# ukeSJTU/tiaozhanbei-unet

Measured on AMD Instinct MI355X. Metric: training images/sec, AnomalyUNet 256x256 bs=32 per GPU, higher is better.
Workload: dtype bf16; 1 GPU; AnomalyUNet 3x256x256, bs=32/GPU, MSE+focal loss, Adam (BASELINE.json configs[2], synthetic randn images, bernoulli masks); global_batch=32, parallelism=dp1, accumulate=fp32, master_params=fp32, dist_world=1, reserved_cus=0, cu_budget=256

## Files before the change

### tiaozhanbei_unet_amd/csrc/igemm.hip

```cpp
#include <stdlib.h>

#include <type_traits>

#include "common.h"

namespace {

struct DView { const char* p; int C, H, W, oy, ox; };
struct DViewW { char* p; int C, H, W, oy, ox; };

struct IgemmParams {
  DView src[2];
  DViewW dst[2];
  int N, H, W;
  int Ctot;
  int Cout;
  int wK;
  const char* w;
  const float* bias;
  int dst_split;
  int accumulate;
  int relu;
  int imul, gtaps;
  int omul, nZ;
  int zdiv;
  float* stats;
  int tilesX, tilesY, nCo;
  const char* bn_y;
  const float* bn_scale;
  const float* bn_shift;
  const float* bn_mean;
  int co_il;
  int pdma_stagger;
  int pdma_dense;
  int pdma_dense_src;
};

constexpr int TH = 8, TW = 16, NPIX = TH * TW;

template <typename T, int TAPS, int BN, int KG>
struct Cfg {
  static constexpr int R = (TAPS == 9) ? 3 : 1;
  static constexpr int HH = TH + R - 1, HW = TW + R - 1;
  static constexpr int CHB = KG * 32;
  static constexpr int PSTR = CHB + 16;
  static constexpr int PPP = CHB / 16;
  static constexpr int A_BUFS = (TAPS == 1) ? 2 : 1;
  static constexpr int A_BYTES = HH * HW * PSTR;
  static constexpr int B_BYTES = BN * PSTR;
  static constexpr int LDS = A_BUFS * A_BYTES + 2 * B_BYTES;
  static constexpr int CK = KG * ET<T>::KGC;
  static constexpr int WCO = BN / 64, WPX = 4 / WCO, PXT = NPIX / (32 * WPX);
  static constexpr int NAP = (HH * HW * PPP + 255) / 256;
  static constexpr int NBP = (BN * PPP + 255) / 256;
  static constexpr bool BN_PIECES_EXACT = (BN * PPP) % 256 == 0;
};

template <typename T, int TAPS, int BN, int KG>
__global__ __launch_bounds__(256, 2) void igemm_kernel(const IgemmParams P) {
  using C = Cfg<T, TAPS, BN, KG>;
  using E = ET<T>;
  extern __shared__ __attribute__((aligned(16))) char smem[];
  char* const sA = smem;
  char* const sB = smem + C::A_BUFS * C::A_BYTES;

  const int tid = threadIdx.x, lane = tid & 63, wave = tid >> 6;
  const int wco = wave % C::WCO, wpx = wave / C::WCO;
  const int l31 = lane & 31, hh = lane >> 5;

  int logical;
  {
    const int total = gridDim.x, b = blockIdx.x;
    const int xcd = b & 7, slot = b >> 3, q = total >> 3, r = total & 7;
    logical = (xcd < r ? xcd * (q + 1) : r * (q + 1) + (xcd - r) * q) + slot;
  }
  const int cot = logical % P.nCo;
  int t = logical / P.nCo;
  const int z = t % P.nZ;  t /= P.nZ;
  const int txi = t % P.tilesX;  t /= P.tilesX;
  const int tyi = t % P.tilesY;
  const int n = t / P.tilesY;
  const int ty0 = tyi * TH, tx0 = txi * TW;
  const int co0 = cot * BN;

  f32x16 acc[2][C::PXT];
#pragma unroll
  for (int a = 0; a < 2; ++a)
#pragma unroll
    for (int b = 0; b < C::PXT; ++b)
#pragma unroll
      for (int r = 0; r < 16; ++r) acc[a][b][r] = 0.f;

  int aoff[2];
#pragma unroll
  for (int ct = 0; ct < 2; ++ct) aoff[ct] = (wco * 64 + ct * 32 + l31) * C::PSTR + hh * 16;
  int boff[C::PXT];
#pragma unroll
  for (int pt = 0; pt < C::PXT; ++pt) {
    const int m = wpx * (32 * C::PXT) + pt * 32 + l31;
    boff[pt] = ((m >> 4) * C::HW + (m & 15)) * C::PSTR + hh * 16;
  }

  const int cpt = P.Ctot / C::CK;
  const int nchunks = P.gtaps * cpt;

  u32x4 breg[C::NBP];
  auto load_b = [&](int tap, int chunk) {
#pragma unroll
    for (int i = 0; i < C::NBP; ++i) {
      const int id = tid + i * 256;
      if (C::BN_PIECES_EXACT || id < BN * C::PPP) {
        const int row = id / C::PPP, part = id % C::PPP;
        const size_t e = ((size_t)((z * TAPS + tap) * P.Cout + co0 + row)) * P.wK + (size_t)chunk * C::CK;
        breg[i] = *reinterpret_cast<const u32x4*>(P.w + e * E::ES + part * 16);
      }
    }
  };
  auto store_b = [&](int buf) {
// ... 642 lines not shown
#pragma unroll
        for (int j = 0; j < 4; ++j) {
          const int cl = wco * 64 + ct * 16 + kb * 4 + j;
          red[(wpx * 2 + 0) * BN + cl] = bs[ct][j];
          red[(wpx * 2 + 1) * BN + cl] = bq[ct][j];
        }
    }
    __syncthreads();
    const int part = (n * P.tilesY + tyi) * P.tilesX + txi;
    for (int i = tid; i < 2 * BN; i += 256) {
      const int q = i / BN, cl = i - q * BN;
      float t = 0.f;
#pragma unroll
      for (int wp = 0; wp < C::WPX; ++wp) t += red[(wp * 2 + q) * BN + cl];
      P.stats[((size_t)part * 2 + q) * P.Cout + co0 + cl] = t;
    }
  }
}

template <typename T, int BN, int KG>
int32_t launch3(const IgemmParams& Pin, int kclass, hipStream_t s, int* stat_parts) {
  using C = Cfg3<T, BN, KG>;
  IgemmParams P = Pin;
  const long long blocks = (long long)P.N * P.tilesY * P.tilesX * P.nCo;
  UNET_REQUIRE(blocks > 0 && blocks < (1LL << 31), UNET_ERR_UNSUPPORTED, "conv3: grid of %lld blocks", blocks);
  const double flops = 2.0 * P.N * P.H * P.W * (double)P.Cout * P.Ctot * 9;
  if constexpr (sizeof(T) == 2 && BN == 128 && KG == 4) {
    using CM = Cfg3M<T, BN, KG>;
    auto km = conv3m16_kernel<T, BN, KG>;
    unet_set_max_lds(reinterpret_cast<const void*>(km), CM::LDS);
    if (P.stats && stat_parts) *stat_parts = P.N * P.tilesY * P.tilesX;
    ProfScope prof(kclass, flops, s, "conv3m16_kernel");
    hipLaunchKernelGGL(km, dim3((unsigned)blocks), dim3(256), CM::LDS, s, P);
    return unet_check_launch("conv3m16_kernel");
  } else {
    auto kern = conv3_kernel<T, BN, KG>;
    unet_set_max_lds(reinterpret_cast<const void*>(kern), C::LDS);
    P.stats = nullptr;
    ProfScope prof(kclass, flops, s, "conv3_kernel");
    hipLaunchKernelGGL(kern, dim3((unsigned)blocks), dim3(256), C::LDS, s, P);
    return unet_check_launch("conv3_kernel");
  }
}

template <int N>
__device__ __forceinline__ void row16_sum_n(float (&v)[N]) {
  static_assert(N >= 3, "hazard distance");
  asm volatile("s_nop 1");
#pragma unroll
  for (int i = 0; i < N; ++i)
    asm volatile("v_add_f32_dpp %0, %1, %1 quad_perm:[1,0,3,2] row_mask:0xf bank_mask:0xf" : "=v"(v[i]) : "0"(v[i]));
#pragma unroll
  for (int i = 0; i < N; ++i)
    asm volatile("v_add_f32_dpp %0, %1, %1 quad_perm:[2,3,0,1] row_mask:0xf bank_mask:0xf" : "=v"(v[i]) : "0"(v[i]));
#pragma unroll
  for (int i = 0; i < N; ++i)
    asm volatile("v_add_f32_dpp %0, %1, %1 row_half_mirror row_mask:0xf bank_mask:0xf" : "=v"(v[i]) : "0"(v[i]));
#pragma unroll
  for (int i = 0; i < N; ++i)
    asm volatile("v_add_f32_dpp %0, %1, %1 row_mirror row_mask:0xf bank_mask:0xf" : "=v"(v[i]) : "0"(v[i]));
}

__device__ __forceinline__ void pdma_item(int wk, int n_tiles, int c, int& cot, int& tile) {
  const int span = c * n_tiles;
  const int sg = wk / span, rem = wk - sg * span;
  tile = rem / c;
  cot = sg * c + (rem - tile * c);
}

template <int BN, bool PAIR = false>
struct CfgP {
  static constexpr int TH = 16, TW = 16, HH = 18, HW = 18;
  static constexpr int PSTR = 160, PPP = 10, RS = HW * PSTR;
  static constexpr int A_INSTR = (HH * HW * PPP + 63) / 64;
  static constexpr int A_BYTES = A_INSTR * 1024;
  static constexpr int NDA = (A_INSTR + 7) / 8;
  static constexpr int W_BYTES = (PAIR ? 2 : 1) * BN * 128, NDW = W_BYTES / 1024 / 8;
  static constexpr int NSLOT = 3;
  static constexpr int W_BASE = 0;
  static constexpr int A_BASE = NSLOT * W_BYTES;
  static constexpr int RED_BASE = A_BASE + 2 * A_BYTES;
  static constexpr int RED_BYTES = 4 * 2 * BN * 4;
  static constexpr int DUMMY = RED_BASE + RED_BYTES;
  static constexpr int LDS = DUMMY + 1024;
  static constexpr int CT = BN / 32;
  static constexpr int NST = CT / 2 * 4;
};

#ifndef PDMA_DEFER128
#define PDMA_DEFER128 (!PP && !BNBWD)
#endif
template <int BN, bool BNBWD = false, bool PP = false, bool PAIR = false>
__device__ __forceinline__ void conv3_pdma_body(const IgemmParams& P) {
  static_assert(!PAIR || (BN == 64 && !PP), "pair steps: the lock-step 64-channel kernel");
  using C = CfgP<BN, PAIR>;
  extern __shared__ __attribute__((aligned(16))) char smem[];
  typedef __attribute__((address_space(3))) void lds_void;
  constexpr unsigned OOB = 0xFFFFFFF0u;

  const int tid = threadIdx.x, lane = tid & 63, wave = tid >> 6;
  const int grp = wave >> 2;
  const int wco = PP ? grp : (wave & 1), wpx = PP ? (wave & 3) : (wave >> 1);
  const int l15 = lane & 15, kb = lane >> 4;

  const int G = gridDim.x;
  const int tiles_img = P.tilesY * P.tilesX;
  const int n_tiles = P.N * tiles_img;
  const int total = n_tiles * P.nCo;
  const int logical = (blockIdx.x & 7) * (G >> 3) + (blockIdx.x >> 3);
  if (logical >= total) return;

  int aoff[C::CT][2], boff[4];
#pragma unroll
  for (int ct = 0; ct < C::CT; ++ct) {
    const int row = wco * (BN / 2) + ct * 16 + l15;
#pragma unroll
    for (int ks = 0; ks < 2; ++ks) aoff[ct][ks] = row * 128 + (((ks * 4 + kb) ^ ((row >> 1) & 7)) << 4);
  }
#pragma unroll
  for (int pt = 0; pt < 4; ++pt) boff[pt] = (wpx * 4 + pt) * C::RS + l15 * C::PSTR + kb * 16;

  int a_code[C::NDA];
#pragma unroll
  for (int j = 0; j < C::NDA; ++j) {
    const int q = (j * 8 + wave) * 64 + lane;
    const int pix = q / C::PPP, part = q - pix * C::PPP;
    const int hy = pix / C::HW, hx = pix - hy * C::HW;
    const int edge = (hy == 0) | ((hy == C::HH - 1) << 1) | ((hx == 0) << 2) | ((hx == C::HW - 1) << 3);
    a_code[j] = (pix < C::HH * C::HW && part < 8) ? (hy | (hx << 8) | (part << 16) | (edge << 24)) : -1;
  }
  unsigned w_g[C::NDW];
#pragma unroll
  for (int j = 0; j < C::NDW; ++j) {
    const int q = (j * 8 + wave) * 64 + lane;
    const int row = q >> 3, pos = q & 7;
    w_g[j] = (unsigned)((row * P.wK) * 2 + ((pos ^ ((row >> 1) & 7)) << 4));
  }

  const int nchunks = P.Ctot / 64;
  const unsigned w_tap_stride = (unsigned)P.Cout * P.wK * 2;
  const __amdgpu_buffer_rsrc_t w_rsrc =
      __builtin_amdgcn_make_buffer_rsrc((void*)P.w, (short)0, (int)(9u * w_tap_stride), 0x00020000);
  const unsigned img0 = (unsigned)P.src[0].H * P.src[0].W * P.src[0].C * 2;
  const unsigned img1 = (unsigned)P.src[1].H * P.src[1].W * P.src[1].C * 2;

  unsigned a_g[2][C::NDA];
  __amdgpu_buffer_rsrc_t a_rsrc[2];
  unsigned d_wbase = 0;
  bool d_live = true;
  const bool dsrc = P.pdma_dense_src != 0;
  if (dsrc) {
#pragma unroll
    for (int j = 0; j < C::NDA; ++j) {
      const int code = a_code[j];
      const int hy = code & 255, hx = (code >> 8) & 255, part = (code >> 16) & 255;
      a_g[1][j] = code >= 0 ? (unsigned)(((hy * P.src[0].W + hx) * P.src[0].C) * 2 + part * 16) : OOB;
    }
  }
  auto setup_dma = [&](int wk) {
    int cot, tile;
    pdma_item(wk, n_tiles, P.co_il, cot, tile);
    const int n = tile / tiles_img, r = tile - n * tiles_img;
    const int ty0 = (r / P.tilesX) * C::TH, tx0 = (r % P.tilesX) * C::TW;
    d_wbase = (unsigned)(cot * BN) * P.wK * 2;
    if (dsrc) {
      const unsigned E = (unsigned)((ty0 == 0) | ((ty0 + C::TH == P.H) << 1) | ((tx0 == 0) << 2) | ((tx0 + C::TW == P.W) << 3)) << 24;
      const long long tb = ((long long)(ty0 - 1) * P.src[0].W + (tx0 - 1)) * (P.src[0].C * 2);
      a_rsrc[0] = __builtin_amdgcn_make_buffer_rsrc((void*)(P.src[0].p + (long long)n * img0 + tb), (short)0, 0x7FFFFFF0, 0x00020000);
      a_rsrc[1] = __builtin_amdgcn_make_buffer_rsrc((void*)(P.src[1].p ? P.src[1].p + (long long)n * img1 + tb : P.src[0].p),
                                                    (short)0, P.src[1].p ? 0x7FFFFFF0 : 0, 0x00020000);
#pragma unroll
      for (int j = 0; j < C::NDA; ++j) a_g[0][j] = ((unsigned)a_code[j] & E) ? OOB : a_g[1][j];
      return;
// ... 114 lines not shown
#pragma unroll
    for (int pt = 0; pt < 4; ++pt) f0[pt] = rb(pbA, 0, pt);
    const bf16x8 a0 = ra(0, 0, 0), a1 = ra(0, 0, 1);
    __builtin_amdgcn_sched_barrier(0);
#pragma unroll
    for (int pt = 0; pt < 4; ++pt) f1[pt] = rb(pbA, 1, pt);
    const bf16x8 a2 = ra(0, 1, 0), a3 = ra(0, 1, 1);
    mm(0, a0, f0);
    mm(1, a1, f0);
    __builtin_amdgcn_sched_barrier(0);
#pragma unroll
    for (int pt = 0; pt < 4; ++pt) g0[pt] = rb(pbB, 0, pt);
    const bf16x8 c0 = ra(1, 0, 0), c1 = ra(1, 0, 1);
    mm(0, a2, f1);
    mm(1, a3, f1);
    __builtin_amdgcn_sched_barrier(0);
#pragma unroll
    for (int pt = 0; pt < 4; ++pt) g1[pt] = rb(pbB, 1, pt);
    const bf16x8 c2 = ra(1, 1, 0), c3 = ra(1, 1, 1);
    mm(0, c0, g0);
    mm(1, c1, g0);
    __builtin_amdgcn_sched_barrier(0);
    mm(0, c2, g1);
    mm(1, c3, g1);
  };

  bf16x8 fa[2][C::CT], fb[2][4];
  auto load_frags = [&](int pbuf, int toff, int slot) {
    const char* pa = smem + C::W_BASE + slot * C::W_BYTES;
    const char* pb = smem + pbuf + toff;
#pragma unroll
    for (int ks = 0; ks < 2; ++ks) {
#pragma unroll
      for (int pt = 0; pt < 4; ++pt) fb[ks][pt] = *reinterpret_cast<const bf16x8*>(pb + boff[pt] + ks * 64);
#pragma unroll
      for (int ct = 0; ct < C::CT; ++ct) fa[ks][ct] = *reinterpret_cast<const bf16x8*>(pa + aoff[ct][ks]);
    }
  };
  auto mma_frags = [&]() {
#pragma unroll
    for (int ks = 0; ks < 2; ++ks)
#pragma unroll
      for (int ct = 0; ct < C::CT; ++ct)
#pragma unroll
        for (int pt = 0; pt < 4; ++pt)
          acc[ct][pt] = __builtin_amdgcn_mfma_f32_16x16x32_bf16(fa[ks][ct], fb[ks][pt], acc[ct][pt], 0, 0, 0);
  };

  setup_dma(logical);
#pragma unroll
  for (int j = 0; j < C::NDA; ++j) dma_patch(0, j, 0, true);
  if constexpr (PAIR) {
    dma_w2(d_wbase, 0, 0, true);
    dma_w2(d_wbase, 2, 1, true);
  } else {
    dma_w(d_wbase, 0, 0, 0, true);
    dma_w(d_wbase, 0, 1, 1, true);
  }
  if constexpr (PP) {
    asm volatile("s_waitcnt vmcnt(%0)" ::"n"(C::NDW) : "memory");
    __builtin_amdgcn_s_barrier();
    if (grp) __builtin_amdgcn_s_barrier();
  }

#ifdef PDMA_STAMPS
  unsigned long long st_sum[4] = {0, 0, 0, 0}, st_prev = 0, st_taps = 0, st_epi = 0, st_b2 = 0, st_rd = 0;
  const unsigned long long st_t0 = __builtin_amdgcn_s_memtime(), st_r0 = __builtin_amdgcn_s_memrealtime();
#endif
  int pbuf_i = 0;
  bool after_epilogue = false;
  const bool late_dma = !PP && P.pdma_stagger && __builtin_amdgcn_readfirstlane(wave) < 4;
  constexpr bool DEFER = BN == 64 || PDMA_DEFER128;
  const bool dense = BNBWD || P.pdma_dense != 0;
  unsigned lp[2];
#pragma unroll
  for (int q = 0; q < 2; ++q)
    lp[q] = (unsigned)((((wpx * 4) * P.dst[q].W + l15) * P.dst[q].C + (kb & 1) * 16 + (kb >> 1) * 8) * 2);
  float stat_tot = 0.f;
  float bs[C::CT][4], bq[C::CT][4];
#pragma unroll
  for (int ct = 0; ct < C::CT; ++ct)
#pragma unroll
    for (int j = 0; j < 4; ++j) { bs[ct][j] = 0.f; bq[ct][j] = 0.f; }
  for (int wk = logical; wk < total; wk += G) {
    int cot, tile;
    pdma_item(wk, n_tiles, P.co_il, cot, tile);
    const int n = tile / tiles_img, r = tile - n * tiles_img;
    const int tyi = r / P.tilesX, txi = r - tyi * P.tilesX;
    const int ty0 = tyi * C::TH, tx0 = txi * C::TW;
    const int co0 = cot * BN;
    const unsigned c_wbase = d_wbase;
    const bool has_next = wk + G < total;
#pragma unroll
    for (int a = 0; a < C::CT; ++a)
#pragma unroll
      for (int b = 0; b < 4; ++b)
#pragma unroll
        for (int q = 0; q < 4; ++q) acc[a][b][q] = 0.f;

    if constexpr (PAIR) {
#pragma unroll
      for (int d = 0; d < 9; ++d) {
        constexpr int NPIECE[9] = {2, 2, 2, 1, 0, 2, 2, 2, 1};
        if (d == 5) {
          d_live = has_next;
          if (has_next) setup_dma(wk + G);
        }
        if (d == 0) {
          if (after_epilogue) {
            if (P.stats) asm volatile("s_waitcnt vmcnt(%0)" ::"n"(C::NDW + C::NST + 1) : "memory");
            else asm volatile("s_waitcnt vmcnt(%0)" ::"n"(C::NDW + C::NST) : "memory");
          } else {
            asm volatile("s_waitcnt vmcnt(%0)" ::"n"(C::NDW) : "memory");
          }
        } else if (d == 4) {
          asm volatile("s_waitcnt vmcnt(%0)" ::"n"(C::NDW) : "memory");
        } else {
          const int np = NPIECE[d == 0 ? 0 : d - 1];
          if (np == 2) asm volatile("s_waitcnt vmcnt(%0)" ::"n"(C::NDW + 2) : "memory");
          else if (np == 1) asm volatile("s_waitcnt vmcnt(%0)" ::"n"(C::NDW + 1) : "memory");
          else asm volatile("s_waitcnt vmcnt(%0)" ::"n"(C::NDW) : "memory");
        }
        __builtin_amdgcn_s_barrier();
        auto issue_dma = [&]() {
          const int first = d < 4 ? 2 * d : 2 * (d - 5);
#pragma unroll
          for (int q = 0; q < NPIECE[d]; ++q) {
            if (d < 4) dma_patch(1, first + q, 1, true);
            else dma_patch(0, first + q, 0, d_live);
          }
          if (d + 2 < 9) dma_w2(c_wbase, 2 * (d + 2), (d + 2) % 3, true);
          else dma_w2(d_wbase, 2 * (d + 2 - 9), (d + 2) % 3, d_live);
        };
        if (!late_dma) issue_dma();
        const int sA = 2 * d, sB = 2 * d + 1;
        const int cA = sA / 9, tA = sA % 9, cB = sB / 9, tB = sB % 9;
        compute2(C::A_BASE + cA * C::A_BYTES, (tA / 3) * C::RS + (tA % 3) * C::PSTR,
                 C::A_BASE + cB * C::A_BYTES, (tB / 3) * C::RS + (tB % 3) * C::PSTR, d % 3);
        if (late_dma) issue_dma();
      }
    } else
    for (int c = 0; c < nchunks; ++c) {
      const bool last = c + 1 == nchunks;
      if (last) {
        d_live = has_next;
        if (has_next) setup_dma(wk + G);
      }
      const int pbuf = C::A_BASE + pbuf_i * C::A_BYTES;
      if constexpr (PP) {
#pragma unroll
        for (int tap = 0; tap < 9; ++tap) {
#ifdef PDMA_STAMPS
          const unsigned long long st_a = __builtin_amdgcn_s_memtime();
          if (st_prev) st_b2 += st_a - st_prev;
#endif
          load_frags(pbuf, (tap / 3) * C::RS + (tap % 3) * C::PSTR, tap % 3);
          __builtin_amdgcn_sched_barrier(0);
#ifdef PDMA_STAMPS
          st_rd += __builtin_amdgcn_s_memtime() - st_a;
#endif
          if (tap < C::NDA) dma_patch(last ? 0 : c + 1, tap, pbuf_i ^ 1, last ? d_live : true);
          if (tap + 2 < 9) dma_w(c_wbase, c, tap + 2, (tap + 2) % 3, true);
          else if (!last) dma_w(c_wbase, c + 1, tap + 2 - 9, (tap + 2) % 3, true);
          else dma_w(d_wbase, 0, tap + 2 - 9, (tap + 2) % 3, d_live);
#ifdef PDMA_STAMPS
          const unsigned long long st_b = __builtin_amdgcn_s_memtime();
          st_sum[0] += st_b - st_a;
#endif
          if (tap == 0 && c == 0 && after_epilogue) {
            if (P.stats) asm volatile("s_waitcnt vmcnt(%0)" ::"n"(1 + C::NDW + C::NST + 1) : "memory");
            else asm volatile("s_waitcnt vmcnt(%0)" ::"n"(1 + C::NDW + C::NST) : "memory");
          } else if (tap < C::NDA) {
            asm volatile("s_waitcnt vmcnt(%0)" ::"n"(1 + C::NDW) : "memory");
          } else {
            asm volatile("s_waitcnt vmcnt(%0)" ::"n"(C::NDW) : "memory");
          }
          asm volatile("s_waitcnt lgkmcnt(0)" ::: "memory");
#ifdef PDMA_STAMPS
          const unsigned long long st_c = __builtin_amdgcn_s_memtime();
          st_sum[1] += st_c - st_b;
#endif
          __builtin_amdgcn_sched_barrier(0);
          __builtin_amdgcn_s_barrier();
          __builtin_amdgcn_sched_barrier(0);
#ifdef PDMA_STAMPS
          const unsigned long long st_d = __builtin_amdgcn_s_memtime();
          st_sum[2] += st_d - st_c;
#endif
          __builtin_amdgcn_s_setprio(1);
          mma_frags();
          __builtin_amdgcn_s_setprio(0);
          __builtin_amdgcn_sched_barrier(0);
#ifdef PDMA_STAMPS
          st_prev = __builtin_amdgcn_s_memtime();
          st_sum[3] += st_prev - st_d;
          st_taps += 1;
#endif
          __builtin_amdgcn_s_barrier();
          __builtin_amdgcn_sched_barrier(0);
        }
      } else {
#pragma unroll
      for (int tap = 0; tap < 9; ++tap) {
#ifdef PDMA_STAMPS
        const unsigned long long st_a = __builtin_amdgcn_s_memtime();
        if (st_prev) st_sum[3] += st_a - st_prev;
#endif
        if (tap == 0 && c == 0 && after_epilogue) {
          if (P.stats) asm volatile("s_waitcnt vmcnt(%0)" ::"n"(C::NDW + C::NST + 1) : "memory");
          else asm volatile("s_waitcnt vmcnt(%0)" ::"n"(C::NDW + C::NST) : "memory");
        } else if (tap == 0 || tap == 8) {
          asm volatile("s_waitcnt vmcnt(%0)" ::"n"(C::NDW) : "memory");
        } else {
          asm volatile("s_waitcnt vmcnt(%0)" ::"n"(C::NDW + 1) : "memory");
        }
#ifdef PDMA_STAMPS
        const unsigned long long st_b = __builtin_amdgcn_s_memtime();
        st_sum[0] += st_b - st_a;
#endif
        __builtin_amdgcn_s_barrier();
#ifdef PDMA_STAMPS
        const unsigned long long st_c = __builtin_amdgcn_s_memtime();
        st_sum[1] += st_c - st_b;
#endif
        auto issue_dma = [&]() {
          if (tap < C::NDA) dma_patch(last ? 0 : c + 1, tap, pbuf_i ^ 1, last ? d_live : true);
          if (tap + 2 < 9) dma_w(c_wbase, c, tap + 2, (tap + 2) % 3, true);
          else if (!last) dma_w(c_wbase, c + 1, tap + 2 - 9, (tap + 2) % 3, true);
          else dma_w(d_wbase, 0, tap + 2 - 9, (tap + 2) % 3, d_live);
        };
        if (!late_dma) issue_dma();
#ifdef PDMA_STAMPS
        st_prev = __builtin_amdgcn_s_memtime();
        st_sum[2] += st_prev - st_c;
        st_taps += 1;
#endif
        compute(pbuf, (tap / 3) * C::RS + (tap % 3) * C::PSTR, tap % 3);
        if (late_dma) issue_dma();
      }
      }
      pbuf_i ^= 1;
    }

#ifdef PDMA_STAMPS
    { const unsigned long long t = __builtin_amdgcn_s_memtime(); if (!PP) st_sum[3] += t - st_prev; st_prev = 0; st_epi -= t; }
#endif
    __amdgpu_buffer_rsrc_t drs[2];
#pragma unroll
    for (int q = 0; q < 2; ++q) {
      const DViewW D = P.dst[q];
      const unsigned dimg = (unsigned)D.H * D.W * D.C * 2u;
      drs[q] = __builtin_amdgcn_make_buffer_rsrc((void*)(D.p ? D.p + (size_t)n * dimg : P.dst[0].p), (short)0,
                                                 D.p ? (int)dimg : 0, 0x00020000);
    }
    if constexpr (!DEFER) {
#pragma unroll
      for (int ct = 0; ct < C::CT; ++ct)
#pragma unroll
        for (int j = 0; j < 4; ++j) { bs[ct][j] = 0.f; bq[ct][j] = 0.f; }
    }
    if constexpr (BNBWD) {
      const DViewW D = P.dst[0];
      const unsigned dimg = (unsigned)D.H * D.W * D.C * 2u;
      const __amdgpu_buffer_rsrc_t yrs =
          __builtin_amdgcn_make_buffer_rsrc((void*)(P.bn_y + (size_t)n * dimg), (short)0, (int)dimg, 0x00020000);
      u32x4 yraw[4][C::CT / 2];
      f32x4 csc[C::CT / 2][2], csh[C::CT / 2][2], cmu[C::CT / 2][2];
      (void)yrs;
      const unsigned rowb = (unsigned)(D.W * D.C * 2);
      __amdgpu_buffer_rsrc_t yrs_c[C::CT / 2], drs_c[C::CT / 2];
#pragma unroll
      for (int cp = 0; cp < C::CT / 2; ++cp) {
        const int cw = co0 + wco * (BN / 2) + cp * 32;
        const unsigned off = (unsigned)(((ty0 * D.W + tx0) * D.C + cw) * 2);
        yrs_c[cp] = __builtin_amdgcn_make_buffer_rsrc((void*)(P.bn_y + (size_t)n * dimg + off), (short)0, (int)(dimg - off), 0x00020000);
        drs_c[cp] = __builtin_amdgcn_make_buffer_rsrc((void*)(D.p + (size_t)n * dimg + off), (short)0, (int)(dimg - off), 0x00020000);
      }
#pragma unroll
      for (int pt = 0; pt < 4; ++pt)
#pragma unroll
        for (int cp = 0; cp < C::CT / 2; ++cp) yraw[pt][cp] = __builtin_amdgcn_raw_buffer_load_b128(yrs_c[cp], lp[0], pt * rowb, 0);
#pragma unroll
      for (int cp = 0; cp < C::CT / 2; ++cp) {
        const int cw = co0 + wco * (BN / 2) + cp * 32 + kb * 4;
#pragma unroll
        for (int t = 0; t < 2; ++t) {
          csc[cp][t] = *reinterpret_cast<const f32x4*>(P.bn_scale + cw + 16 * t);
          csh[cp][t] = *reinterpret_cast<const f32x4*>(P.bn_shift + cw + 16 * t);
          cmu[cp][t] = *reinterpret_cast<const f32x4*>(P.bn_mean + cw + 16 * t);
        }
      }
#pragma unroll
      for (int pt = 0; pt < 4; ++pt) {
#pragma unroll
        for (int cp = 0; cp < C::CT / 2; ++cp) {
          const u32x4 o = yraw[pt][cp];
          const auto o0 = __builtin_amdgcn_permlane16_swap(o[0], o[2], false, false);
          const auto o1 = __builtin_amdgcn_permlane16_swap(o[1], o[3], false, false);
          const bf16x4 ya = __builtin_bit_cast(bf16x4, u32x2{o0[0], o1[0]});
          const bf16x4 yb = __builtin_bit_cast(bf16x4, u32x2{o0[1], o1[1]});
          bf16x4 ra, rb;
#pragma unroll
          for (int j = 0; j < 4; ++j) {
            const float fa = (float)ya[j], fb = (float)yb[j];
            const bool ona = fmaf(fa, csc[cp][0][j], csh[cp][0][j]) > 0.f;
            const bool onb = fmaf(fb, csc[cp][1][j], csh[cp][1][j]) > 0.f;
            ra[j] = (bf16_t)(ona ? acc[2 * cp][pt][j] : 0.f);
            rb[j] = (bf16_t)(onb ? acc[2 * cp + 1][pt][j] : 0.f);
            const float qa = (float)ra[j], qb = (float)rb[j];
            bs[2 * cp][j] += qa;
            bq[2 * cp][j] = fmaf(qa, fa - cmu[cp][0][j], bq[2 * cp][j]);
            bs[2 * cp + 1][j] += qb;
            bq[2 * cp + 1][j] = fmaf(qb, fb - cmu[cp][1][j], bq[2 * cp + 1][j]);
          }
          const u32x2 ua = __builtin_bit_cast(u32x2, ra), ub = __builtin_bit_cast(u32x2, rb);
          const auto s0 = __builtin_amdgcn_permlane16_swap(ua[0], ub[0], false, false);
          const auto s1 = __builtin_amdgcn_permlane16_swap(ua[1], ub[1], false, false);
          __builtin_amdgcn_raw_buffer_store_b128(u32x4{s0[0], s1[0], s0[1], s1[1]}, drs_c[cp], lp[0], pt * rowb, 0);
        }
      }
    } else {
    auto finish = [&](int pt, int cp, int cw, bool second, int accq, __amdgpu_buffer_rsrc_t rs, unsigned vo, unsigned so, bool ok) {
      float va[4], vb[4];
#pragma unroll
      for (int j = 0; j < 4; ++j) { va[j] = acc[2 * cp][pt][j]; vb[j] = acc[2 * cp + 1][pt][j]; }
      if (P.bias) {
        const float* bp = P.bias + cw + kb * 4;
#pragma unroll
        for (int j = 0; j < 4; ++j) { va[j] += bp[j]; vb[j] += bp[16 + j]; }
      }
      if (P.relu) {
#pragma unroll
        for (int j = 0; j < 4; ++j) { va[j] = fmaxf(va[j], 0.f); vb[j] = fmaxf(vb[j], 0.f); }
      }
      if (accq) {
        const u32x4 o = __builtin_amdgcn_raw_buffer_load_b128(rs, vo, so, 0);
        const auto o0 = __builtin_amdgcn_permlane16_swap(o[0], o[2], false, false);
        const auto o1 = __builtin_amdgcn_permlane16_swap(o[1], o[3], false, false);
        const bf16x4 oa = __builtin_bit_cast(bf16x4, u32x2{o0[0], o1[0]});
        const bf16x4 ob = __builtin_bit_cast(bf16x4, u32x2{o0[1], o1[1]});
#pragma unroll
        for (int j = 0; j < 4; ++j) { va[j] += (float)oa[j]; vb[j] += (float)ob[j]; }
      }
      bf16x4 ra, rb;
#pragma unroll
      for (int j = 0; j < 4; ++j) { ra[j] = (bf16_t)va[j]; rb[j] = (bf16_t)vb[j]; }
      const u32x2 ua = __builtin_bit_cast(u32x2, ra), ub = __builtin_bit_cast(u32x2, rb);
      const auto s0 = __builtin_amdgcn_permlane16_swap(ua[0], ub[0], false, false);
      const auto s1 = __builtin_amdgcn_permlane16_swap(ua[1], ub[1], false, false);
      __builtin_amdgcn_raw_buffer_store_b128(u32x4{s0[0], s1[0], s0[1], s1[1]}, rs, vo, so, 0);
      if (ok && P.stats) {
#pragma unroll
        for (int j = 0; j < 4; ++j) {
          const float qa = (float)ra[j], qb = (float)rb[j];
          bs[2 * cp][j] += qa;
          bq[2 * cp][j] = fmaf(qa, qa, bq[2 * cp][j]);
          bs[2 * cp + 1][j] += qb;
          bq[2 * cp + 1][j] = fmaf(qb, qb, bq[2 * cp + 1][j]);
        }
      }
    };
    if (dense) {
#pragma unroll
      for (int cp = 0; cp < C::CT / 2; ++cp) {
        const int cw = co0 + wco * (BN / 2) + cp * 32;
        const bool second = cw >= P.dst_split;
        const int accq = second ? (P.accumulate & 2) : (P.accumulate & 1);
        const DViewW D = second ? P.dst[1] : P.dst[0];
        const unsigned dimg = (unsigned)D.H * D.W * D.C * 2u;
        const unsigned off = (unsigned)(((ty0 * D.W + tx0) * D.C + cw - (second ? P.dst_split : 0)) * 2);
        const __amdgpu_buffer_rsrc_t rs =
            __builtin_amdgcn_make_buffer_rsrc((void*)(D.p + (size_t)n * dimg + off), (short)0, (int)(dimg - off), 0x00020000);
        const unsigned rowb = (unsigned)(D.W * D.C * 2);
        const unsigned lpq = second ? lp[1] : lp[0];
#pragma unroll
        for (int pt = 0; pt < 4; ++pt) finish(pt, cp, cw, second, accq, rs, lpq, pt * rowb, true);
      }
    } else {
#pragma unroll
      for (int pt = 0; pt < 4; ++pt) {
        const int fy = ty0 + wpx * 4 + pt, fx = tx0 + l15;
        const bool pix_ok = fy < P.H && fx < P.W;
#pragma unroll
        for (int cp = 0; cp < C::CT / 2; ++cp) {
          const int cw = co0 + wco * (BN / 2) + cp * 32;
          const bool second = cw >= P.dst_split;
          const int accq = second ? (P.accumulate & 2) : (P.accumulate & 1);
          const DViewW D = second ? P.dst[1] : P.dst[0];
          const int co = cw - (second ? P.dst_split : 0) + (kb & 1) * 16 + (kb >> 1) * 8;
          const int y = fy - D.oy, x = fx - D.ox;
          const bool ok = pix_ok && y >= 0 && y < D.H && x >= 0 && x < D.W;
          const unsigned vo = ok ? (unsigned)(((y * D.W + x) * D.C + co) * 2) : OOB;
          if (second) finish(pt, cp, cw, true, accq, drs[1], vo, 0u, ok);
          else finish(pt, cp, cw, false, accq, drs[0], vo, 0u, ok);
        }
      }
    }
    }
    if (P.stats) {
      int ncot = cot, ntile_ = 0;
      if (has_next) pdma_item(wk + G, n_tiles, P.co_il, ncot, ntile_);
      (void)ntile_;
      const bool flush = !P.zdiv || !has_next || ncot != cot;
      const int part = P.zdiv ? logical / P.co_il : (n * P.tilesY + tyi) * P.tilesX + txi;
      float tsum = 0.f;
      unsigned so = OOB;
      if (!DEFER || flush) {
        {
          float rv[2 * C::CT * 4];
#pragma unroll
          for (int ct = 0; ct < C::CT; ++ct)
#pragma unroll
            for (int j = 0; j < 4; ++j) { rv[ct * 4 + j] = bs[ct][j]; rv[C::CT * 4 + ct * 4 + j] = bq[ct][j]; }
          row16_sum_n(rv);
#pragma unroll
          for (int ct = 0; ct < C::CT; ++ct)
#pragma unroll
            for (int j = 0; j < 4; ++j) { bs[ct][j] = rv[ct * 4 + j]; bq[ct][j] = rv[C::CT * 4 + ct * 4 + j]; }
        }
        float* red = reinterpret_cast<float*>(smem + C::RED_BASE);
        if (l15 == 0) {
#pragma unroll
          for (int ct = 0; ct < C::CT; ++ct)
#pragma unroll
            for (int j = 0; j < 4; ++j) {
              const int cl = wco * (BN / 2) + ct * 16 + kb * 4 + j;
              red[(wpx * 2 + 0) * BN + cl] = bs[ct][j];
              red[(wpx * 2 + 1) * BN + cl] = bq[ct][j];
            }
        }
#pragma unroll
        for (int ct = 0; ct < C::CT; ++ct)
#pragma unroll
          for (int j = 0; j < 4; ++j) { bs[ct][j] = 0.f; bq[ct][j] = 0.f; }
        asm volatile("s_waitcnt lgkmcnt(0)" ::: "memory");
        __builtin_amdgcn_s_barrier();
        const int st_t = PP ? (tid & 255) : tid;
        if (st_t < (PP ? BN : 2 * BN)) {
          const int q = PP ? st_t / (BN / 2) : st_t / BN;
          const int cl = PP ? grp * (BN / 2) + st_t % (BN / 2) : st_t - q * BN;
#pragma unroll
          for (int wp = 0; wp < 4; ++wp) tsum += red[(wp * 2 + q) * BN + cl];
          if (!DEFER && P.zdiv) {
            stat_tot += tsum;
            tsum = stat_tot;
            if (flush) stat_tot = 0.f;
          }
          if (flush) so = (unsigned)((((size_t)part * 2 + q) * P.Cout + co0 + cl) * 4);
        }
      }
      const __amdgpu_buffer_rsrc_t srs = __builtin_amdgcn_make_buffer_rsrc(
          (void*)P.stats, (short)0, (int)std::min<long long>((long long)n_tiles * 2 * P.Cout * 4, 0x7FFFFFFFLL), 0x00020000);
      __builtin_amdgcn_raw_buffer_store_b32(__builtin_bit_cast(unsigned, tsum), srs, so, 0, 0);
    }
    after_epilogue = true;
#ifdef PDMA_STAMPS
    st_epi += __builtin_amdgcn_s_memtime();
#endif
  }
#ifdef PDMA_STAMPS
  if (P.bn_mean && lane == 0) {
    unsigned long long* o = (unsigned long long*)P.bn_mean + ((size_t)blockIdx.x * 8 + wave) * 8;
    o[0] = st_sum[0]; o[1] = st_sum[1]; o[2] = st_sum[2]; o[3] = st_sum[3]; o[4] = st_taps; o[5] = PP ? st_rd : st_epi;
    o[6] = st_b2;
    o[7] = ((__builtin_amdgcn_s_memtime() - st_t0) << 20) / (__builtin_amdgcn_s_memrealtime() - st_r0 + 1);
  }
#endif
  if constexpr (PP) { if (!grp) __builtin_amdgcn_s_barrier(); }
  asm volatile("s_waitcnt vmcnt(0)" ::: "memory");
}

__global__ __launch_bounds__(512, 1) void conv3_pdma128_kernel(const IgemmParams P) { conv3_pdma_body<128>(P); }
__global__ __launch_bounds__(512, 1) void conv3_pdma64_kernel(const IgemmParams P) { conv3_pdma_body<64>(P); }
__global__ __launch_bounds__(512, 1) void conv3_pdma128_bnbwd_kernel(const IgemmParams P) { conv3_pdma_body<128, true>(P); }
__global__ __launch_bounds__(512, 1) void conv3_pdma64_bnbwd_kernel(const IgemmParams P) { conv3_pdma_body<64, true>(P); }
__global__ __launch_bounds__(512, 1) void conv3_pp128_kernel(const IgemmParams P) { conv3_pdma_body<128, false, true>(P); }
__global__ __launch_bounds__(512, 1) void conv3_pp64_kernel(const IgemmParams P) { conv3_pdma_body<64, false, true>(P); }
__global__ __launch_bounds__(512, 1) void conv3_pp128_bnbwd_kernel(const IgemmParams P) { conv3_pdma_body<128, true, true>(P); }
__global__ __launch_bounds__(512, 1) void conv3_pp64_bnbwd_kernel(const IgemmParams P) { conv3_pdma_body<64, true, true>(P); }
__global__ __launch_bounds__(512, 1) void conv3_pdma64x2_kernel(const IgemmParams P) { conv3_pdma_body<64, false, false, true>(P); }
__global__ __launch_bounds__(512, 1) void conv3_pdma64x2_bnbwd_kernel(const IgemmParams P) { conv3_pdma_body<64, true, false, true>(P); }

#ifdef PDMA_STAMPS
void* g_pdma_debug = nullptr;
#endif

template <int BN>
int32_t launch_pdma(const IgemmParams& Pin, int kclass, hipStream_t s, int* stat_parts) {
  using C = CfgP<BN>;
  IgemmParams P = Pin;
  P.nCo = P.Cout / BN;
  P.tilesX = cdiv(P.W, C::TW);
  P.tilesY = cdiv(P.H, C::TH);
  const bool bnbwd = P.bn_y != nullptr;
  P.pdma_stagger = 1;
  P.pdma_dense = 1;
  P.pdma_dense_src = 1;
  for (int k = 0; k < 2; ++k)
    if (P.src[k].p && P.src[k].C > 0 &&
        (P.src[k].oy || P.src[k].ox || P.src[k].H != P.H || P.src[k].W != P.W || P.src[k].C != P.src[0].C))
      P.pdma_dense_src = 0;
  for (int q = 0; q < 2; ++q)
    if (P.dst[q].p && (P.dst[q].oy || P.dst[q].ox || P.dst[q].H != P.H || P.dst[q].W != P.W)) P.pdma_dense = 0;
  const bool pp = BN == 128 && P.Ctot >= 512;
  const bool pair = BN == 64 && P.Ctot == 128;
  auto kern = pair ? (bnbwd ? conv3_pdma64x2_bnbwd_kernel : conv3_pdma64x2_kernel)
              : pp ? (bnbwd ? (BN == 128 ? conv3_pp128_bnbwd_kernel : conv3_pp64_bnbwd_kernel)
                            : (BN == 128 ? conv3_pp128_kernel : conv3_pp64_kernel))
                   : (bnbwd ? (BN == 128 ? conv3_pdma128_bnbwd_kernel : conv3_pdma64_bnbwd_kernel)
                            : (BN == 128 ? conv3_pdma128_kernel : conv3_pdma64_kernel));
  const int lds_bytes = pair ? CfgP<64, true>::LDS : C::LDS;
  unet_set_max_lds(reinterpret_cast<const void*>(kern), lds_bytes);
  const long long work = (long long)P.N * P.tilesY * P.tilesX * P.nCo;
  UNET_REQUIRE(work > 0 && work < (1LL << 30), UNET_ERR_UNSUPPORTED, "conv3_pdma: %lld work items", work);
  const long long stat_bytes = (long long)P.N * P.tilesY * P.tilesX * 2 * P.Cout * 4;
  if (stat_bytes >= 0x7FFFFFFFLL) {
    UNET_REQUIRE(!bnbwd, UNET_ERR_UNSUPPORTED, "conv3_pdma: partial-sum buffer of %lld bytes", stat_bytes);
    P.stats = nullptr;
  }
  const int blocks = (int)std::min<long long>(unet_cu_budget(), cdiv64(work, 8) * 8);
  const double flops = 2.0 * P.N * P.H * P.W * (double)P.Cout * P.Ctot * 9;
  const long long n_tiles = (long long)P.N * P.tilesY * P.tilesX;
  P.co_il = 1;
  while (P.co_il * 2 <= 4 && P.nCo % (P.co_il * 2) == 0 && blocks % (P.co_il * 2 * 8) == 0) P.co_il *= 2;
  P.zdiv = (P.stats && (n_tiles * P.co_il) % blocks == 0) ? 1 : 0;
  if (P.stats && stat_parts) *stat_parts = P.zdiv ? blocks / P.co_il : (int)n_tiles;
#ifdef PDMA_STAMPS
  if (!bnbwd) P.bn_mean = (const float*)g_pdma_debug;
#endif
  const double px = (double)P.N * P.H * P.W;
  const double alg_bytes = 2.0 * (px * (P.Ctot + P.Cout * (1.0 + (bnbwd ? 1 : 0) + (P.accumulate ? 1 : 0))) + 9.0 * P.Ctot * P.Cout);
  ProfScope prof(kclass, flops, s, bnbwd ? (BN == 128 ? "conv3_pdma128_bnbwd_kernel" : "conv3_pdma64_bnbwd_kernel")
                                          : (BN == 128 ? "conv3_pdma128_kernel" : "conv3_pdma64_kernel"), alg_bytes);
  hipLaunchKernelGGL(kern, dim3((unsigned)blocks), dim3(512), lds_bytes, s, P);
  return unet_check_launch("conv3_pdma_kernel");
}

struct CfgWS {
  static constexpr int WTH = 16, WTW = 16;
  static constexpr int HH = WTH + 2, HW = WTW + 2;
  static constexpr int PSTR = 128 + 16;
  static constexpr int RS = (HW * PSTR + 255) / 256 * 256;
  static constexpr int PIECES = HH * (RS / 16);
  static constexpr int NWAVE = 8;
  static constexpr int NINSTR = (PIECES + 63) / 64;
  static constexpr int NDMA = (NINSTR + NWAVE - 1) / NWAVE;
  static constexpr int A_BYTES = NINSTR * 1024;
  static constexpr int NBUF = 3;
  static constexpr int RED_BASE = NBUF * A_BYTES + 1024;
  static constexpr int RED_BYTES = 2 * 2 * 8 * 64 * 4;
  static constexpr int CT_BASE = RED_BASE + RED_BYTES;
  static constexpr int LDS = CT_BASE + 3 * 64 * 4;
  static constexpr int PXT = 2;
  static constexpr int ROWS = 64;
};

template <bool ACC, int STATS = 0>
__global__ __launch_bounds__(512, 1) void conv3_ws_kernel(const IgemmParams P, int tiles_per_block) {
  using C = CfgWS;
  constexpr bool ST = STATS == 1;
  static_assert(!(ACC && STATS), "the gradient fan-in form carries no statistics");
  extern __shared__ __attribute__((aligned(16))) char smem[];
  const int tid = threadIdx.x, lane = tid & 63, wave = tid >> 6;
  const int grp = wave >> 2;
  const int wco = ST ? grp : (wave & 1), wpx = ST ? (wave & 3) : (wave >> 1);
  const int l31 = lane & 31, hh = lane >> 5;
  const int nCg = P.Cout / C::ROWS;
  const int xcd = blockIdx.x & 7, slot = blockIdx.x >> 3;
  const int cg = slot % nCg, tr = (slot / nCg) * 8 + xcd;
  const int co_lane = cg * C::ROWS + wco * 32 + l31;
  const int tiles_img = P.tilesX * P.tilesY;
  const int total_tiles = P.N * tiles_img;
  const int t_begin = tr * tiles_per_block;
  const int t_end = min(t_begin + tiles_per_block, total_tiles);
  if (t_begin >= t_end) {
    if (STATS && tid < 128)
      P.stats[((size_t)tr * 2 + (tid >> 6)) * P.Cout + cg * C::ROWS + (tid & 63)] = 0.f;
    return;
  }
  float* const red = reinterpret_cast<float*>(smem + C::RED_BASE);
  float* const ctab = reinterpret_cast<float*>(smem + C::CT_BASE);
  if (STATS == 2 && tid < 192) {
    const float* srcp = tid < 64 ? P.bn_scale : (tid < 128 ? P.bn_shift : P.bn_mean);
    ctab[tid] = srcp[cg * C::ROWS + (tid & 63)];
  }
  float stat_tot = 0.f;

  bf16x8 wreg[36];
  {
    const bf16_t* wp = reinterpret_cast<const bf16_t*>(P.w);
#pragma unroll
    for (int tap = 0; tap < 9; ++tap)
#pragma unroll
      for (int kg = 0; kg < 4; ++kg)
        wreg[tap * 4 + kg] = *reinterpret_cast<const bf16x8*>(wp + ((size_t)(tap * P.Cout + co_lane)) * P.wK + kg * 16 + hh * 8);
    __builtin_amdgcn_s_waitcnt(0x0F70);
  }

  int boff[C::PXT];
#pragma unroll
  for (int pt = 0; pt < C::PXT; ++pt) {
    const int m = wpx * (32 * C::PXT) + pt * 32 + l31;
    boff[pt] = (m >> 4) * C::RS + (m & 15) * C::PSTR + hh * 16;
  }
  constexpr unsigned OOB = 0xFFFFFFF0u;
  const DView S = P.src[0];
  unsigned a_pk[(C::NDMA + 1) / 2];
#pragma unroll
  for (int j = 0; j < C::NDMA; ++j) {
    const int q = (j * C::NWAVE + wave) * 64 + lane;
    const int hy = q / (C::RS / 16), rem = q - hy * (C::RS / 16);
// ... 1501 lines not shown
```

Baseline: 1841 images/sec.

## Prefetch BN-backward y tiles during last taps and stage BN coefficients in LDS

In the BN-backward variant of the pipelined 3x3 conv kernel, the y tile is now prefetched via buffer-load-to-LDS during the final two taps of the last channel chunk, with adjusted vmcnt waits. Per-channel scale/shift/mean coefficients are loaded once per output-channel tile into a new LDS region instead of being re-read from global memory in every epilogue. The DEFER path is also enabled for BN-backward 128-channel kernels. The goal is to hide epilogue global-load latency; the cost is extra LDS, an added barrier whenever the channel tile changes, and more delicate waitcnt accounting.

```diff
diff --git a/tiaozhanbei_unet_amd/csrc/igemm.hip b/tiaozhanbei_unet_amd/csrc/igemm.hip
--- a/tiaozhanbei_unet_amd/csrc/igemm.hip
+++ b/tiaozhanbei_unet_amd/csrc/igemm.hip
@@ -34,6 +34,9 @@
   int pdma_stagger;
   int pdma_dense;
   int pdma_dense_src;
+#ifdef PDMA_STAMPS
+  void* pdma_dbg;
+#endif
 };
 
 constexpr int TH = 8, TW = 16, NPIX = TH * TW;
@@ -842,13 +845,15 @@
   static constexpr int RED_BASE = A_BASE + 2 * A_BYTES;
   static constexpr int RED_BYTES = 4 * 2 * BN * 4;
   static constexpr int DUMMY = RED_BASE + RED_BYTES;
-  static constexpr int LDS = DUMMY + 1024;
+  static constexpr int COEF_BASE = DUMMY + 1024;
+  static constexpr int LDS = COEF_BASE + 3 * BN * 4;
   static constexpr int CT = BN / 32;
   static constexpr int NST = CT / 2 * 4;
+  static constexpr int NPF = NST / 2;
 };
 
 #ifndef PDMA_DEFER128
-#define PDMA_DEFER128 (!PP && !BNBWD)
+#define PDMA_DEFER128 (!PP)
 #endif
 template <int BN, bool BNBWD = false, bool PP = false, bool PAIR = false>
 __device__ __forceinline__ void conv3_pdma_body(const IgemmParams& P) {
@@ -1129,6 +1134,10 @@
   for (int ct = 0; ct < C::CT; ++ct)
 #pragma unroll
     for (int j = 0; j < 4; ++j) { bs[ct][j] = 0.f; bq[ct][j] = 0.f; }
+  int coef_cot = -1;
+  const int cf_t = PP ? (tid & 255) : tid;
+  const int cf_q = PP ? cf_t / (BN / 2) : cf_t / BN;
+  const int cf_cl = PP ? grp * (BN / 2) + cf_t % (BN / 2) : cf_t - cf_q * BN;
   for (int wk = logical; wk < total; wk += G) {
     int cot, tile;
     pdma_item(wk, n_tiles, P.co_il, cot, tile);
@@ -1136,6 +1145,26 @@
     const int tyi = r / P.tilesX, txi = r - tyi * P.tilesX;
     const int ty0 = tyi * C::TH, tx0 = txi * C::TW;
     const int co0 = cot * BN;
+    const bool coef_new = BNBWD && cot != coef_cot;
+    float coef_v = 0.f;
+    if constexpr (BNBWD) {
+      if (coef_new && cf_q < 3) coef_v = (cf_q == 0 ? P.bn_scale : (cf_q == 1 ? P.bn_shift : P.bn_mean))[co0 + cf_cl];
+      coef_cot = cot;
+    }
+    auto prefetch_y = [&](int half) {
+      const DViewW D = P.dst[0];
+      const unsigned dimg = (unsigned)D.H * D.W * D.C * 2u;
+      const unsigned off = (unsigned)(((ty0 * D.W + tx0) * D.C + co0 + wco * (BN / 2)) * 2);
+      const unsigned rowb = (unsigned)(D.W * D.C * 2);
+      const __amdgpu_buffer_rsrc_t yrs_p =
+          __builtin_amdgcn_make_buffer_rsrc((void*)(P.bn_y + (size_t)n * dimg + off), (short)0, (int)(dimg - off), 0x00020000);
+#pragma unroll
+      for (int r2 = 0; r2 < 2; ++r2)
+#pragma unroll
+        for (int cp = 0; cp < C::CT / 2; ++cp)
+          __builtin_amdgcn_raw_ptr_buffer_load_lds(yrs_p, (lds_void*)(smem + C::DUMMY), 16, lp[0],
+                                                   (unsigned)(half * 2 + r2) * rowb + cp * 64, 0, 0);
+    };
     const unsigned c_wbase = d_wbase;
     const bool has_next = wk + G < total;
 #pragma unroll
@@ -1210,6 +1239,7 @@
           if (tap + 2 < 9) dma_w(c_wbase, c, tap + 2, (tap + 2) % 3, true);
           else if (!last) dma_w(c_wbase, c + 1, tap + 2 - 9, (tap + 2) % 3, true);
           else dma_w(d_wbase, 0, tap + 2 - 9, (tap + 2) % 3, d_live);
+          if constexpr (BNBWD) { if (last && tap >= 7) prefetch_y(tap - 7); }
 #ifdef PDMA_STAMPS
           const unsigned long long st_b = __builtin_amdgcn_s_memtime();
           st_sum[0] += st_b - st_a;
@@ -1219,6 +1249,9 @@
             else asm volatile("s_waitcnt vmcnt(%0)" ::"n"(1 + C::NDW + C::NST) : "memory");
           } else if (tap < C::NDA) {
             asm volatile("s_waitcnt vmcnt(%0)" ::"n"(1 + C::NDW) : "memory");
+          } else if (BNBWD && last) {
+            if (tap == 7) asm volatile("s_waitcnt vmcnt(%0)" ::"n"(C::NDW + C::NPF) : "memory");
+            else asm volatile("s_waitcnt vmcnt(%0)" ::"n"(C::NDW + 2 * C::NPF) : "memory");
           } else {
             asm volatile("s_waitcnt vmcnt(%0)" ::"n"(C::NDW) : "memory");
           }
@@ -1256,6 +1289,8 @@
         if (tap == 0 && c == 0 && after_epilogue) {
           if (P.stats) asm volatile("s_waitcnt vmcnt(%0)" ::"n"(C::NDW + C::NST + 1) : "memory");
           else asm volatile("s_waitcnt vmcnt(%0)" ::"n"(C::NDW + C::NST) : "memory");
+        } else if (BNBWD && tap == 8 && last) {
+          asm volatile("s_waitcnt vmcnt(%0)" ::"n"(C::NDW + C::NPF) : "memory");
         } else if (tap == 0 || tap == 8) {
           asm volatile("s_waitcnt vmcnt(%0)" ::"n"(C::NDW) : "memory");
         } else {
@@ -1275,6 +1310,7 @@
           if (tap + 2 < 9) dma_w(c_wbase, c, tap + 2, (tap + 2) % 3, true);
           else if (!last) dma_w(c_wbase, c + 1, tap + 2 - 9, (tap + 2) % 3, true);
           else dma_w(d_wbase, 0, tap + 2 - 9, (tap + 2) % 3, d_live);
+          if constexpr (BNBWD) { if (last && tap >= 7) prefetch_y(tap - 7); }
         };
         if (!late_dma) issue_dma();
 #ifdef PDMA_STAMPS
@@ -1327,20 +1363,23 @@
       for (int pt = 0; pt < 4; ++pt)
 #pragma unroll
         for (int cp = 0; cp < C::CT / 2; ++cp) yraw[pt][cp] = __builtin_amdgcn_raw_buffer_load_b128(yrs_c[cp], lp[0], pt * rowb, 0);
+      float* cf = reinterpret_cast<float*>(smem + C::COEF_BASE);
+      if (coef_new) {
+        if (cf_q < 3) cf[cf_q * BN + cf_cl] = coef_v;
+        asm volatile("s_waitcnt lgkmcnt(0)" ::: "memory");
+        __builtin_amdgcn_s_barrier();
+      }
 #pragma unroll
       for (int cp = 0; cp < C::CT / 2; ++cp) {
-        const int cw = co0 + wco * (BN / 2) + cp * 32 + kb * 4;
+        const int cw = wco * (BN / 2) + cp * 32 + kb * 4;
 #pragma unroll
         for (int t = 0; t < 2; ++t) {
-          csc[cp][t] = *reinterpret_cast<const f32x4*>(P.bn_scale + cw + 16 * t);
-          csh[cp][t] = *reinterpret_cast<const f32x4*>(P.bn_shift + cw + 16 * t);
-          cmu[cp][t] = *reinterpret_cast<const f32x4*>(P.bn_mean + cw + 16 * t);
-        }
-      }
-#pragma unroll
-      for (int pt = 0; pt < 4; ++pt) {
-#pragma unroll
-        for (int cp = 0; cp < C::CT / 2; ++cp) {
+          csc[cp][t] = *reinterpret_cast<const f32x4*>(cf + cw + 16 * t);
+          csh[cp][t] = *reinterpret_cast<const f32x4*>(cf + BN + cw + 16 * t);
+          cmu[cp][t] = *reinterpret_cast<const f32x4*>(cf + 2 * BN + cw + 16 * t);
+        }
+#pragma unroll
+        for (int pt = 0; pt < 4; ++pt) {
           const u32x4 o = yraw[pt][cp];
           const auto o0 = __builtin_amdgcn_permlane16_swap(o[0], o[2], false, false);
           const auto o1 = __builtin_amdgcn_permlane16_swap(o[1], o[3], false, false);
@@ -1506,9 +1545,9 @@
 #endif
   }
 #ifdef PDMA_STAMPS
-  if (P.bn_mean && lane == 0) {
-    unsigned long long* o = (unsigned long long*)P.bn_mean + ((size_t)blockIdx.x * 8 + wave) * 8;
-    o[0] = st_sum[0]; o[1] = st_sum[1]; o[2] = st_sum[2]; o[3] = st_sum[3]; o[4] = st_taps; o[5] = PP ? st_rd : st_epi;
+  if (P.pdma_dbg && lane == 0) {
+    unsigned long long* o = (unsigned long long*)P.pdma_dbg + ((size_t)blockIdx.x * 8 + wave) * 8;
+    o[0] = st_sum[0]; o[1] = st_sum[1]; o[2] = st_sum[2]; o[3] = st_sum[3]; o[4] = st_taps; o[5] = (PP && !BNBWD) ? st_rd : st_epi;
     o[6] = st_b2;
     o[7] = ((__builtin_amdgcn_s_memtime() - st_t0) << 20) / (__builtin_amdgcn_s_memrealtime() - st_r0 + 1);
   }
@@ -1573,7 +1612,7 @@
   P.zdiv = (P.stats && (n_tiles * P.co_il) % blocks == 0) ? 1 : 0;
   if (P.stats && stat_parts) *stat_parts = P.zdiv ? blocks / P.co_il : (int)n_tiles;
 #ifdef PDMA_STAMPS
-  if (!bnbwd) P.bn_mean = (const float*)g_pdma_debug;
+  P.pdma_dbg = g_pdma_debug;
 #endif
   const double px = (double)P.N * P.H * P.W;
   const double alg_bytes = 2.0 * (px * (P.Ctot + P.Cout * (1.0 + (bnbwd ? 1 : 0) + (P.accumulate ? 1 : 0))) + 9.0 * P.Ctot * P.Cout);
```

Result: no change. 1841 images/sec (-0.0%).
